# zrjer/Sparse-Matrix-Factorization-Library

Measured on AMD Instinct MI355X. Metric: numeric-factorization GFLOP/s (supernodal Cholesky), higher is better.
Workload: dtype f64; 1 GPU; 3D 7-point Laplacian 128^3 SPD Cholesky fp64, geometric ND, devSlotSize 8694792192; n=2097152, nnz_input=8339456, nsuper=35419, factor_doubles=3787034536, parallelism=single GPU, grid_rule=BASELINE config

## Files before the change

sparse-matrix-factorization-library_amd/csrc/sf_chol_plan.hip:

```cpp
#include <sparseframe_hip.h>

#include <algorithm>
#include <time.h>
#include <cmath>
#include <cstdio>
#include <cstdlib>
#include <cstring>
#include <string>
#include <vector>

#include "sf_plan_internal.h"
#include "sf_symbolic.h"

extern "C" {

int sf_device_count(void) {
    int n = 0;
    if (hipGetDeviceCount(&n) != hipSuccess) return 0;
    return n;
}

size_t sf_device_memory(int device) {
    hipDeviceProp_t prop;
    if (hipGetDeviceProperties(&prop, device) != hipSuccess) return 0;
// ... 199 lines not shown
                if (p->lu) sf::launch_getrf(p->d_potrf + L.first, L.count, p->d_Lsx, p->xC, p->d_info, pc, st);
                else sf::launch_potrf(p->d_potrf + L.first, L.count, p->d_Lsx, p->d_info, st);
                break;
            case 1: sf::launch_trsm(p->d_trsm + L.first, L.count, p->d_Lsx, pc.pivinv, st); break;
            case 7: {
                const int g = (int)L.first;
                const int upto = p->ooc_wait.empty() ? g - 2 : p->ooc_wait[(size_t)g];
                for (int w = std::max(0, g - 2); w <= upto && w < g; ++w) {
                    std::unique_lock<std::mutex> lk(p->dl_mu);
                    p->dl_cv.wait(lk, [&] { return p->dl_abort || p->dl_group_left[(size_t)w].load() <= 0; });
                    if (p->dl_abort) return SF_ERR_HIP;
                }
                if (g >= 2 && p->ooc_buf > 0) {
                    const size_t off = (size_t)(g & 1) * (size_t)p->ooc_buf, nb = (size_t)p->ooc_buf * sizeof(double);
                    HIP_TRY(hipMemsetAsync(p->d_Lsx + off, 0, nb, st));
                    if (p->lu) HIP_TRY(hipMemsetAsync(p->d_Lsx + p->xC + off, 0, nb, st));
                }
                if (p->ooc_top_mode >= 1)
                    for (const auto& z : p->ooc_zero[(size_t)g]) {
                        HIP_TRY(hipMemsetAsync(p->d_Lsx + z.first, 0, (size_t)z.second * sizeof(double), st));
                        if (p->lu) HIP_TRY(hipMemsetAsync(p->d_Lsx + p->xC + z.first, 0, (size_t)z.second * sizeof(double), st));
                    }
                assemble(p->d_loadmask + (size_t)g * (size_t)p->nsuper, st);
                break;
            }
            case 6: {
                int64_t lo, hi;
                launch_window(L, L.count, &lo, &hi);
                sf::launch_update_small(p->d_probs, p->d_stasks + L.first + lo, (int)(hi - lo), p->d_Lsx, p->d_relmap, st);
                break;
            }
            case 5:
                sf::launch_step(p->d_steps + L.first, L.count, p->lu ? 1 : 0, p->d_Lsx, p->d_flags, p->epoch, p->d_info, p->d_tinv,
                                p->d_info + 1 + L.ticket, pc, st);
                break;
            case 2:
            case 3:
            case 4: {
                int64_t w0, w1;
                launch_window(L, L.units, &w0, &w1);
                const uint32_t u0 = (uint32_t)w0, u1 = (uint32_t)w1;
                sf::launch_gemm(p->d_probs, p->d_gtasks + L.first, p->d_ktprefix + L.prefix_first, L.count, u0, u1,
                                L.kind == 3 ? 1 : 0, p->d_Lsx, p->d_relmap, p->gemm_dynamic ? p->d_info + 1 + L.ticket : nullptr, st,
                                (L.whole_tiles && !L.split) ? 1 : 0, 0);
                break;
            }
        }
        if (p->profiling) { kinds.push_back(L.kind); mark(); }
        if (p->dl_active) HIP_TRY(dl_publish(p, li + 1));
    }
    if (last && !p->capturing) HIP_TRY(hipEventRecord(p->ev1, st));
    HIP_TRY(hipGetLastError());
    if (p->profiling) {
        HIP_TRY(hipStreamSynchronize(st));
        if (first) {
            p->last_load_ms = p->last_panel_ms = p->last_update_ms = 0;
            for (double& v : p->last_kind_ms) v = 0;
        }
        float ms = 0;
        if (first && !evs.empty() && elapsed_ms(&ms, p->ev0, evs[0])) p->last_load_ms = ms;
        FILE* dump = nullptr;
        if (const char* path = getenv("SF_PROFILE_DUMP")) dump = fopen(path, first ? "w" : "a");
        if (dump && first) fprintf(dump, "launch,kind,tasks,units,flops,ms\n");
        for (size_t k = 0; k + 1 < evs.size(); ++k) {
            if (!elapsed_ms(&ms, evs[k], evs[k + 1])) continue;
            if (kinds[k] == 3) p->last_update_ms += ms; else if (kinds[k] != 6) p->last_panel_ms += ms;
            p->last_kind_ms[kinds[k]] += ms;
// ... 750 lines not shown

int sf_chol_plan_set_profiling(sf_chol_plan* p, int on) {
    if (!p) return SF_ERR_ARG;
    p->profiling = on != 0;
    return SF_OK;
}

double sf_chol_plan_stat(const sf_chol_plan* p, const char* name) {
    if (!p || !name) return -1;
    const std::string k(name);
    if (k == "levels") return p->nlevels;
    if (k == "last_solve_ms") return p->last_solve_ms;
    if (k == "last_solve_many_ms") return p->last_solve_many_ms;
    if (k == "bytes_solve_many") return (double)p->bytes_solve_many;
    if (k == "solve_many_width") return (double)sf::SVM_W;
    if (k == "bytes_selinv") return (double)p->bytes_selinv;
    if (k == "last_selinv_ms") return p->last_selinv_ms;
    if (k == "flops_selinv") return p->flops_selinv;
    if (k == "selinv_valid") return (p->d_sel && p->sel_gen == p->factor_gen) ? 1.0 : 0.0;
    if (k == "last_refine_iters") return (double)p->last_refine_iters;
    if (k == "last_refine_berr0") return p->last_refine_berr0;
    if (k == "last_refine_berr") return p->last_refine_berr;
    if (k == "last_refine_ms") return p->last_refine_ms;
    if (k == "last_residual_ms") return p->last_residual_ms;
    if (k == "bytes_refine") return (double)p->bytes_refine;
    if (k == "refine_row_entries") return (double)p->rf_entries;
    if (k == "perturbed_pivots") return (double)p->last_perturbed;
    if (k == "pivot_tol") return p->piv_tol;
    if (k == "last_to_host_ms") return p->last_to_host_ms;
    if (k == "download_pieces") return (double)p->dl_pieces.size();
    if (k == "top_doubles") return (double)p->top_size;
    if (k == "stored_doubles") return (double)p->xC;
    if (k == "launches") return (double)p->launches.size();
    if (k == "gemm_tasks") return (double)p->n_gemm_tasks;
    if (k == "update_pairs") return (double)p->n_pairs;
    if (k == "flops_exec") return p->flops_exec;
    if (k == "flops_update") return p->flops_update;
    if (k == "flops_panel_gemm") return p->flops_panel_gemm;
    if (k == "scatter_elems") return p->scatter_elems;
    if (k == "bytes_device") return (double)p->bytes_device;
    if (k == "last_ms") return p->last_ms;
    if (k == "last_load_ms") return p->last_load_ms;
    if (k == "last_panel_ms") return p->last_panel_ms;
    if (k == "last_update_ms") return p->last_update_ms;
    if (k == "last_potrf_ms") return p->last_kind_ms[0];
    if (k == "last_trsm_ms") return p->last_kind_ms[1];
    if (k == "last_inner_gemm_ms") return p->last_kind_ms[2];
    if (k == "last_outer_gemm_ms") return p->last_kind_ms[4];
    if (k == "last_step_ms") return p->last_kind_ms[5];
    if (k == "last_small_update_ms") return p->last_kind_ms[6];
    if (k == "flops_update_small") return p->flops_update_small;
    if (k == "flops_outer_gemm") return p->flops_outer_gemm;
    if (k == "flops_tiles") return p->flops_tiles;
    if (k == "flops_tiles_update") return p->flops_tiles_update;
    return -1;
}

}
```

sparse-matrix-factorization-library_amd/csrc/sf_kernels.h:

```cpp
#pragma once
#include <hip/hip_runtime.h>
#include <cstdint>

#include <cstdlib>
static inline const char* sf_exp_env(const char* name) {
#ifdef SF_EXPERIMENTS
    return getenv(name);
#else
    (void)name;
    return nullptr;
#endif
}

namespace sf {

constexpr int NB = 64;
constexpr int OUTER_NB = 512;
constexpr int TRSM_ROWS = 256;
constexpr int ST_ROWS = 64;
constexpr int GEMM_BM = 128;
constexpr int GEMM_BN = 128;
constexpr int GEMM_BK = 16;
constexpr int GEMM_WAVES = 8;
constexpr int GEMM_THREADS = 64 * GEMM_WAVES;
// ... 33 lines not shown
struct PotrfTask {
    int64_t panel;
    int32_t ld, diag, b;
    int32_t first_col;
};

struct PivotCtl {
    double tol, eps;
    int32_t* pivpos;
    int32_t* pivinv;
    int* nperturb;
};

struct TrsmTask {
    int64_t panel;
    int64_t dpanel;
    int32_t ld, diag, b;
    int32_t row0, nrows;
    int32_t unit;
    int32_t first_col;
    int32_t pad;
};

struct StepTask {
    int64_t panel;
    int64_t xpanel;
    int32_t ld, J, diag, b;
    int32_t row0, nrows;
    int32_t flag;
    int32_t mode;
    int32_t slot;
    int32_t next_b;
    int32_t first_col;
    int32_t pad;
};

void launch_build_loadmap(const int64_t* Lp, const int32_t* Li, int32_t n, const int32_t* Super, const int32_t* SuperMap,
                          const int64_t* Lsip, const int32_t* Lsi, const int64_t* Lsxp, int64_t base, int skip_diag, int64_t* map, hipStream_t st);
void launch_loadmap_drop(const int64_t* drop, int64_t count, int64_t* map, hipStream_t st);
void launch_load_mapped(const double* Lx, const int64_t* map, int64_t nnz, double* Lsx, hipStream_t st);
void launch_load_panels(const int64_t* Lp, const int32_t* Li, const double* Lx, int32_t n,
                        const int32_t* Super, const int32_t* SuperMap, const int64_t* Lsip, const int32_t* Lsi,
                        const int64_t* Lsxp, double* Lsx, int skip_diag, const int8_t* load_mask, hipStream_t st);
void launch_potrf(const PotrfTask* tasks, int ntasks, double* Lsx, int* info, hipStream_t st);
void launch_getrf(const PotrfTask* tasks, int ntasks, double* Lsx, int64_t u_shift, int* info, PivotCtl pc, hipStream_t st);
struct FillTile { int64_t xp; int32_t nsrow, r0, c0, cb, ce; };
void launch_factor_hash(const int32_t* Super, const int64_t* Lsip, const int64_t* Xp, const int64_t* RefXp, int32_t nsuper,
                        const double* PL, const double* PU, int lu, int64_t total, unsigned long long* H, hipStream_t st);
void launch_lu_fill_u11(const FillTile* tiles, int64_t ntiles, double* PL, const double* PU, hipStream_t st);
void launch_pack_lu(const int32_t* Super, const int64_t* Lsip, const int64_t* Xp, const int64_t* RefXp, int32_t nsuper,
                    const double* PL, const double* PU, double* out, int64_t e_begin, int64_t e_end, hipStream_t st);
void launch_trsm(const TrsmTask* tasks, int ntasks, double* Lsx, const int32_t* pivinv, hipStream_t st);
void launch_step(const StepTask* tasks, int ntasks, int lu, double* Lsx, int* flags, int epoch, int* info, double* tinv, int* ticket,
                 PivotCtl pc, hipStream_t st);
void launch_build_relmaps(const GemmProb* probs, int nprobs, const int32_t* Lsi, int32_t* RelMap, hipStream_t st);

void launch_gemm(const GemmProb* probs, const GemmTask* tasks, const uint32_t* kt_prefix, int ntasks, uint32_t u_lo, uint32_t u_hi,
                 int mode, double* Lsx, const int32_t* RelMap, int* ticket, hipStream_t st, int whole_tiles = 0, int grid_cap = 0);

void launch_update_small(const GemmProb* probs, const GemmTask* tasks, int ntasks, double* Lsx, const int32_t* RelMap, hipStream_t st);

struct SolveTask {
    int64_t panel;
    int64_t rows;
    int32_t ld, diag, b;
    int32_t row0, nrows;
    int32_t first_col;
    int32_t flag;
    int32_t expect;
    int64_t tdiag;
};
constexpr int SVM_W = 16;
void launch_solve_small_fwd(const SolveTask* t, int nt, int width, const double* Lsx, const int32_t* Lsi, double* x, int unit,
                            const int32_t* pivpos, hipStream_t st);
void launch_solve_small_bwd(const SolveTask* t, int nt, int width, const double* Lsx, const int32_t* Lsi, double* x, hipStream_t st);
void launch_solve_fwd(const SolveTask* t, int nt, int width, int big, const double* Lsx, const int32_t* Lsi, double* x, int unit,
                      const int32_t* pivpos, int* sync, int* ticket, int* info, hipStream_t st);
void launch_solve_bwd(const SolveTask* t, int nt, int width, int big, const double* Lsx, const int32_t* Lsi, double* x, int* sync, int* ticket,
                      int* info, hipStream_t st, const double* Tbase = nullptr);
void launch_solve_transpose_diag(const SolveTask* tasks, const int64_t* list, int64_t ntasks, const double* Lsx, double* T, hipStream_t st);

void launch_solve_many_pack(const double* Bc, int64_t n, int cw, double* X, hipStream_t st);
void launch_solve_many_unpack(const double* X, int64_t n, int cw, double* Bc, hipStream_t st);

struct SelUnit {
    int64_t lx, rows;
    int32_t nsrow, ncol, cb, w;
// ... 28 lines not shown
```

sparse-matrix-factorization-library_amd/csrc/sf_plan_build.hip:

```cpp
#include <sparseframe_hip.h>

#include <algorithm>
#include <time.h>
#include <cmath>
#include <cstdio>
#include <cstdlib>
#include <cstring>
#include <vector>

#include "sf_plan_internal.h"
#include "sf_symbolic.h"

static thread_local double* t_offer_ptr = nullptr;
static thread_local size_t t_offer_bytes = 0;
extern "C" void sf_plan_offer_factor_buffer(double* ptr, size_t bytes) { t_offer_ptr = ptr; t_offer_bytes = bytes; }

struct PlanInput {
    sf_long n = 0, nsuper = 0;
    const sf_long *Super = nullptr, *SuperMap = nullptr, *Lsip = nullptr, *Lsi = nullptr, *Lsxp = nullptr;
    const sf_long *Lp = nullptr, *Li = nullptr, *Up = nullptr, *Ui = nullptr;
    bool lu = false;
    int device = 0;
    bool dry = false;
    const int32_t* phase_in = nullptr;
    int load_top = 1, rank = 0, nranks = 1;
    const uint32_t* top_mask = nullptr;
    const double* root_cum = nullptr;
    const int32_t* ooc_group = nullptr;
    int ooc_ngroups = 0, ooc_top_mode = 0;

    sf_long nscol(sf_long s) const { return Super[s + 1] - Super[s]; }
    sf_long nsrow(sf_long s) const { return Lsip[s + 1] - Lsip[s]; }
    bool ooc() const { return ooc_group != nullptr && ooc_ngroups > 1; }
    int sides() const { return lu ? 2 : 1; }
};

static bool exp_on(const char* name) {
    const char* env = sf_exp_env(name);
    return !(env && atoi(env) == 0);
}

struct PlanKnobs {
    bool trace = false;
    int su_maxk = sf::SU_MAXK;
    int64_t fuse_max = 32 * sf::GEMM_GRID;
    bool lookahead = true;
    bool use_graph = false;
    bool top_owner = false;
    bool solve_diagT = true, solve_bwd_ahead = true, solve_bwd_fused = true, solve_fwd_ahead = true, solve_fwd_far_first = true;
    int solve_far_wgs = 512, solve_far_groups = 8;
    int dl_workers = DL_WORKERS_DEFAULT, dl_workers_fresh = DL_WORKERS_FRESH;
    bool dl_host_wait = true;
    int64_t dl_slot = DL_SLOT_DEFAULT;
    bool dl_2d = true;
    bool dl_lu_pack = false;
    bool stream_priority = true;
    bool gemm_dynamic = true;
    double piv_tol = 0.0, piv_perturb = 0.0;
};

static PlanKnobs read_knobs() {
    PlanKnobs k;
    k.trace = getenv("SF_TRACE") != nullptr;
    if (const char* env = sf_exp_env("SF_SU_MAXK")) k.su_maxk = atoi(env);
    if (const char* env = getenv("SF_FUSE_MAX")) k.fuse_max = strtoll(env, nullptr, 10);
    if (const char* env = getenv("SF_LOOKAHEAD")) k.lookahead = atoi(env) != 0;
    if (const char* env = getenv("SF_GRAPH")) k.use_graph = atoi(env) != 0;
    if (const char* env = getenv("SF_TOP_OWNER")) k.top_owner = atoi(env) != 0;
    k.solve_diagT = exp_on("SF_SOLVE_DIAGT");
    k.solve_bwd_ahead = exp_on("SF_SOLVE_BWD_AHEAD");
    k.solve_bwd_fused = exp_on("SF_SOLVE_BWD_FUSED");
    k.solve_fwd_ahead = exp_on("SF_SOLVE_FWD_AHEAD");
    k.solve_fwd_far_first = exp_on("SF_SOLVE_FWD_FAR_FIRST");
    if (const char* env = sf_exp_env("SF_SOLVE_FAR_WGS")) k.solve_far_wgs = std::max(1, atoi(env));
    if (const char* env = sf_exp_env("SF_SOLVE_FAR_GROUPS")) k.solve_far_groups = std::max(1, std::min(64, atoi(env)));
    if (const char* env = getenv("SF_DL_WORKERS")) k.dl_workers = k.dl_workers_fresh = std::max(1, std::min(DL_WORKERS_MAX, atoi(env)));
    k.dl_host_wait = exp_on("SF_DL_HOST_WAIT");
    if (const char* env = getenv("SF_DL_SLOT_MB")) k.dl_slot = (int64_t)std::max(1, atoi(env)) << 17;
    k.dl_2d = exp_on("SF_DL_2D");
    if (const char* env = sf_exp_env("SF_DL_LU_PACK")) k.dl_lu_pack = atoi(env) != 0;
    k.stream_priority = exp_on("SF_STREAM_PRIORITY");
    k.gemm_dynamic = exp_on("SF_GEMM_DYNAMIC");
    if (const char* env = getenv("SF_LU_PIVOT_TOL")) {
        k.piv_tol = std::min(1.0, std::max(0.0, atof(env)));
        if (k.piv_tol > 0.0) k.piv_perturb = 1.4901161193847656e-08;
    }
    if (const char* env = getenv("SF_LU_PERTURB")) k.piv_perturb = std::max(0.0, atof(env));
    return k;
}

struct Layout {
    std::vector<int64_t> XP;
    std::vector<uint32_t> gmask;
    int64_t ushift = 0;
    uint32_t all_ranks = 1;
    int rank = 0;
    int group_idx(uint32_t m) const { return __builtin_popcount(m & ((1u << rank) - 1u)); }
};
// ... 400 lines not shown

static void reduce_point(const PlanInput& in, const Layout& lay, const LevelSet& LS, sf_chol_plan& p, int jo, bool ahead) {
    const int J = jo * sf::OUTER_NB;
    if (!p.segments.empty()) p.segments.back().l1 = p.launches.size();
    Segment sg;
    sg.mask = LS.mask;
    sg.l0 = p.launches.size();
    for (sf_long s : LS.sn) {
        const int64_t nscol = in.nscol(s), nsrow = in.nsrow(s);
        if (J >= nscol) continue;
        const int64_t w = std::min<int64_t>(sf::OUTER_NB, nscol - J);
        for (int side = 0; side < in.sides(); ++side) {
            const int64_t base = lay.XP[s] + (side ? lay.ushift : 0);
            sg.off.push_back(base + (int64_t)J * nsrow);
            sg.cnt.push_back(w * nsrow);
            sg.src.push_back(base + (int64_t)J * nsrow + J);
            sg.rows.push_back(nsrow - J);
            sg.cols.push_back(w);
            sg.ld.push_back(nsrow);
            sg.packed += (nsrow - J) * w;
        }
    }
    sg.early = ahead && jo > 0;
    if (p.top_owner && ahead && LS.share_cnt == in.nranks) sg.owner_gi = jo % LS.share_cnt;
    p.segments.push_back(std::move(sg));
}

struct SweepState {
    bool split_set = false;
    int ooc_open = -1;
    std::vector<int32_t> pre_updated;
};

static int fused_step(const PlanInput& in, const Layout& lay, const LevelSet& LS, SweepState& sw, PlanTables& T, sf_chol_plan& p,
                      int jo, int ti, int diag) {
    const bool lu = in.lu;
    const int J = jo * sf::OUTER_NB, ninner = sf::OUTER_NB / sf::NB;
    const int64_t ushift = lay.ushift;
    const std::vector<int64_t>& XP = lay.XP;
    std::vector<StepTask>& steps = T.steps;
    const int64_t d0 = (int64_t)steps.size();
    std::vector<int32_t> flag_of, slot_of;
    for (sf_long s : LS.sn) {
        const int nscol = (int)in.nscol(s), nsrow = (int)in.nsrow(s);
        if (diag >= nscol) { flag_of.push_back(-1); slot_of.push_back(-1); continue; }
        const int b = std::min(sf::NB, nscol - diag);
        flag_of.push_back(T.n_flags);
        if (lu && ti >= 2 && sw.pre_updated[(size_t)s] != jo * 16 + ti) {
            fprintf(stderr, "[sparseframe-hip] plan_create: LU step %d of outer block %d of supernode %lld has no pre-update task\n", ti, jo, (long long)s);
            return SF_ERR_ARG;
        }
        steps.push_back(StepTask{XP[s], XP[s] + (lu ? ushift : 0), nsrow, lu ? (ti >= 2 ? diag - sf::NB : J) : diag, diag, b, diag, b, T.n_flags++, 0, (int32_t)(steps.size() - d0), 0, (int32_t)in.Super[s], 0});
        slot_of.push_back((int32_t)(steps.size() - 1 - d0));
        if (ti > 0) p.flops_panel_gemm += (lu ? 2.0 : 1.0) * ((double)b * (b + 1) * (diag - J) + 2.0 * (nsrow - diag - b) * (double)b * (diag - J));
    }
    if (lu && ti >= 1 && ti + 1 < ninner) {
        const int dnext = diag + sf::NB;
        for (sf_long s : LS.sn) {
            const int nscol = (int)in.nscol(s), nsrow = (int)in.nsrow(s);
            if (dnext >= nscol) continue;
            const int bn = std::min(sf::NB, nscol - dnext);
            steps.push_back(StepTask{XP[s], XP[s] + ushift, nsrow, J, dnext, bn, dnext, bn, -1, 2, 0, 0, (int32_t)in.Super[s], 0});
            sw.pre_updated[(size_t)s] = jo * 16 + ti + 1;
        }
    }
    size_t si = 0;
    for (sf_long s : LS.sn) {
        const int nscol = (int)in.nscol(s), nsrow = (int)in.nsrow(s);
        const int32_t fl = flag_of[si], sl = slot_of[si];
        ++si;
        if (fl < 0) continue;
        const int b = std::min(sf::NB, nscol - diag);
        for (int r = diag + b; r < nsrow; r += sf::ST_ROWS) {
            const int nr = std::min(sf::ST_ROWS, nsrow - r);
            if (!lu) {
                const int nb = (r < std::min(nscol, J + sf::OUTER_NB)) ? std::min(sf::NB, nscol - r) : 0;
                steps.push_back(StepTask{XP[s], XP[s], nsrow, J, diag, b, r, nr, fl, 0, sl, nb, (int32_t)in.Super[s], 0});
            } else {
                steps.push_back(StepTask{XP[s], XP[s] + ushift, nsrow, J, diag, b, r, nr, fl, 0, sl, 0, (int32_t)in.Super[s], 0});
                steps.push_back(StepTask{XP[s] + ushift, XP[s], nsrow, J, diag, b, r, nr, fl, 1, sl, 0, (int32_t)in.Super[s], 0});
            }
        }
    }
    if ((int64_t)steps.size() > d0) {
        p.launches.push_back(Launch{5, d0, (int)(steps.size() - d0)});
        p.launches.back().ticket = p.n_tickets++;
    }
    T.max_diag_tasks = std::max<int64_t>(T.max_diag_tasks, (int64_t)slot_of.size());
    return SF_OK;
}

static void three_launch_step(const PlanInput& in, const Layout& lay, const LevelSet& LS, PlanTables& T, sf_chol_plan& p, int J, int diag) {
    const std::vector<int64_t>& XP = lay.XP;
    const int64_t ushift = lay.ushift;
    const int64_t p0 = (int64_t)T.potrf.size(), t0 = (int64_t)T.trsm.size(), g0 = (int64_t)T.gtasks.size();
    for (sf_long s : LS.sn) {
        const int nscol = (int)in.nscol(s), nsrow = (int)in.nsrow(s);
        if (diag >= nscol) continue;
        const int b = std::min(sf::NB, nscol - diag);
        if (diag > J) {
            GemmProb g{};
            g.lda = nsrow; g.ldc = nsrow;
            g.M = nsrow - diag; g.N = b; g.K = diag - J;
            const int64_t src = XP[s] + diag + (int64_t)J * nsrow;
            const int64_t dst = XP[s] + diag + (int64_t)diag * nsrow;
            const int32_t first = push_sides(in, lay, T, g, src, dst);
            for (int32_t id = first; id < (int32_t)T.probs.size(); ++id) {
                p.flops_panel_gemm += (double)g.N * (g.N + 1) * g.K + 2.0 * (g.M - g.N) * (double)g.N * g.K;
                add_tiles(T, p, id);
            }
        }
        T.potrf.push_back(PotrfTask{XP[s], nsrow, diag, b, (int32_t)in.Super[s]});
        const int below = diag + b;
        for (int r = below; r < nsrow; r += sf::TRSM_ROWS) {
            const int nr = std::min(sf::TRSM_ROWS, nsrow - r);
            if (!in.lu) {
                T.trsm.push_back(TrsmTask{XP[s], XP[s], nsrow, diag, b, r, nr, 0, (int32_t)in.Super[s], 0});
            } else {
                T.trsm.push_back(TrsmTask{XP[s], XP[s] + ushift, nsrow, diag, b, r, nr, 0, (int32_t)in.Super[s], 0});
// ... 78 lines not shown
        p.launches.back().flops = level_small_flops;
    }
}

static int schedule_set(const PlanInput& in, const PlanKnobs& kn, const Layout& lay, const LevelSet& LS, SweepState& sw, PlanTables& T,
                        sf_chol_plan& p) {
    if (LS.ph == 1 && !sw.split_set) { p.launch_split = p.launches.size(); sw.split_set = true; }
    while (in.ooc() && LS.group > sw.ooc_open) p.launches.push_back(Launch{7, (int64_t)++sw.ooc_open, 0});
    const bool shared = set_is_shared(in, LS);
    sf_long maxcol = 0;
    for (sf_long s : LS.sn) maxcol = std::max(maxcol, in.nscol(s));
    const int nouter = (int)((maxcol + sf::OUTER_NB - 1) / sf::OUTER_NB);
    const bool ahead = shared && p.lookahead && LS.share_cnt > 1;
    constexpr int KT_BLOCK = sf::OUTER_NB / sf::GEMM_BK;
    for (int jo = 0; jo < nouter; ++jo) {
        const int J = jo * sf::OUTER_NB;
        if (jo > 0 && !ahead) outer_gemm(in, lay, LS, T, p, J, 0, -1, shared);
        if (shared) {
            reduce_point(in, lay, LS, p, jo, ahead);
            if (ahead && jo > 0) outer_gemm(in, lay, LS, T, p, J, (jo - 1) * KT_BLOCK, jo * KT_BLOCK, false);
        }
        const int ninner = sf::OUTER_NB / sf::NB;
        bool block_fused = false;
        for (int ti = 0; ti < ninner; ++ti) {
            const int diag = J + ti * sf::NB;
            if (diag >= maxcol) break;
            int64_t step_wgs = 0;
            for (sf_long s : LS.sn) {
                const int64_t nscol = in.nscol(s), nsrow = in.nsrow(s);
                if (diag < nscol) step_wgs += 1 + in.sides() * ((nsrow - std::min<int64_t>(nscol, diag + sf::NB) + sf::ST_ROWS - 1) / sf::ST_ROWS);
            }
            if (ti == 0) block_fused = step_wgs <= kn.fuse_max;
            if (!block_fused) three_launch_step(in, lay, LS, T, p, J, diag);
            else if (int rc = fused_step(in, lay, LS, sw, T, p, jo, ti, diag)) return rc;
        }
        const bool owner_block = shared && !p.segments.empty() && p.segments.back().owner_gi >= 0;
        if (owner_block) p.segments.back().lc = p.launches.size();
        for (sf_long s : LS.sn)
            if (J < in.nscol(s)) T.blk_ready[T.blk_first[s] + jo] = p.launches.size() + (owner_block ? 1 : 0);
        if (ahead && jo + 2 < nouter) outer_gemm(in, lay, LS, T, p, J + 2 * sf::OUTER_NB, 0, (jo + 1) * KT_BLOCK, true);
    }
    schur_updates(in, kn, lay, LS, T, p);
    return SF_OK;
}

static int schedule_factorization(const PlanInput& in, const PlanKnobs& kn, const Layout& lay, const std::vector<LevelSet>& sets,
                                  PlanTables& T, sf_chol_plan& p) {
    T.blk_first.assign(in.nsuper + 1, 0);
    for (sf_long s = 0; s < in.nsuper; ++s) T.blk_first[s + 1] = T.blk_first[s] + (in.nscol(s) + sf::OUTER_NB - 1) / sf::OUTER_NB;
    T.blk_ready.assign(T.blk_first[in.nsuper], 0);
    p.lookahead = kn.lookahead;
    p.use_graph = kn.use_graph;
    p.top_owner = kn.top_owner && !in.lu;
    SweepState sw;
    sw.pre_updated.assign(in.lu ? (size_t)std::max<sf_long>(in.nsuper, 1) : 0, -1);
    p.launch_split = 0;
    for (const LevelSet& LS : sets)
        if (int rc = schedule_set(in, kn, lay, LS, sw, T, p)) return rc;
    if (!sw.split_set) p.launch_split = p.launches.size();
    if (!p.segments.empty()) p.segments.back().l1 = p.launches.size();
    p.n_gemm_tasks = (int64_t)T.gtasks.size() + (int64_t)T.stasks.size();
    return SF_OK;
}

static void schedule_solve(const PlanInput& in, const PlanKnobs& kn, const Layout& lay, PlanTables& T, sf_chol_plan& p) {
    int32_t n_solve_sync = 0;
    const bool solve_mapped = p.partial && in.top_mask != nullptr && in.load_top == 2;
// ... 745 lines not shown
```

sparse-matrix-factorization-library_amd/csrc/sf_plan_internal.h:

```cpp
#pragma once
#include <sparseframe_hip.h>

#include <algorithm>
#include <atomic>
#include <condition_variable>
#include <cstdio>
#include <cstdlib>
#include <memory>
#include <mutex>
#include <thread>
#include <utility>
#include <vector>

#include "sf_kernels.h"

using sf::GemmProb;
using sf::GemmTask;
using sf::PotrfTask;
using sf::TrsmTask;
using sf::StepTask;

struct Launch {
    int kind;
    int64_t first;
    int count;
    int64_t prefix_first = 0;
    uint32_t units = 0;
    double flops = 0;
    bool split = false;
    int share_idx = 0, share_cnt = 1;
    bool whole_tiles = false;
    double share_lo = 0.0, share_hi = 1.0;
    int ticket = 0;
};

struct Segment {
    uint32_t mask = 0;
    size_t l0 = 0, l1 = 0;
    std::vector<int64_t> off, cnt;
    std::vector<int64_t> src, rows, cols, ld;
    int64_t packed = 0;
    bool early = false;
    int owner_gi = -1;
    size_t lc = 0;
};

#define HIP_TRY(expr)                                                                       \
    do {                                                                                    \
        hipError_t e_ = (expr);                                                             \
        if (e_ != hipSuccess) {                                                             \
            fprintf(stderr, "[sparseframe-hip] %s failed: %s (%s:%d)\n", #expr, hipGetErrorString(e_), __FILE__, __LINE__); \
            return SF_ERR_HIP;                                                              \
        }                                                                                   \
    } while (0)

template <class T>
static inline int upload(T** dptr, const std::vector<T>& h, size_t* bytes_total) {
    *dptr = nullptr;
    const size_t bytes = std::max<size_t>(h.size(), 1) * sizeof(T);
    HIP_TRY(hipMalloc((void**)dptr, bytes));
    if (!h.empty()) HIP_TRY(hipMemcpy(*dptr, h.data(), h.size() * sizeof(T), hipMemcpyHostToDevice));
    *bytes_total += bytes;
    return SF_OK;
}

constexpr int64_t DL_SLOT_DEFAULT = (int64_t)4 << 20;
// ... 142 lines not shown
    std::vector<SelStep> sel_steps;
    std::vector<sf::SelPair> sel_pairs_h;
    int64_t sel_linv_elems = 0, sel_y_elems = 0, sel_z_elems = 0, sel_s_elems = 0;
    double* d_sel = nullptr;
    double* d_sel_diag = nullptr;
    void* d_sel_units = nullptr;
    void* d_sel_pairs = nullptr;
    double* d_sel_scratch = nullptr;
    size_t bytes_selinv = 0;
    double last_selinv_ms = 0, flops_selinv = 0;
    int64_t *d_rf_ptr = nullptr, *d_rf_pos = nullptr, *d_rf_cptr = nullptr, *d_rf_cpos = nullptr;
    int32_t *d_rf_col = nullptr, *d_rf_ccol = nullptr;
    double* d_rf_vec = nullptr;
    int64_t rf_entries = 0, rf_anorm_gen = -1;
    size_t bytes_refine = 0;
    int last_refine_iters = 0;
    double last_refine_berr0 = 0, last_refine_berr = 0, last_refine_ms = 0, last_residual_ms = 0;
    int device = 0;
    int64_t n = 0, nsuper = 0, nnz = 0, isize = 0, xsize = 0;
    hipStream_t stream = nullptr;
    hipEvent_t ev0 = nullptr, ev1 = nullptr, ev_s0 = nullptr, ev_s1 = nullptr;

    int64_t* d_Lp = nullptr;
    int32_t* d_Li = nullptr;
    double* d_Lx = nullptr;
    int32_t* d_Super = nullptr;
    int32_t* d_SuperMap = nullptr;
    int64_t* d_Lsip = nullptr;
    int32_t* d_Lsi = nullptr;
    int64_t* d_Lsxp = nullptr;
    double* d_Lsx = nullptr;
    int* d_info = nullptr;
    int n_tickets = 0;
    bool gemm_dynamic = true;

    PotrfTask* d_potrf = nullptr;
    TrsmTask* d_trsm = nullptr;
    StepTask* d_steps = nullptr;
    int* d_flags = nullptr;
    double* d_tinv = nullptr;
    int epoch = 0;
    std::vector<uint64_t> h_hash;
    int hash_epoch = -1;
    GemmProb* d_probs = nullptr;
    GemmTask* d_gtasks = nullptr;
    GemmTask* d_stasks = nullptr;
    uint32_t* d_ktprefix = nullptr;
    int32_t* d_relmap = nullptr;

    std::vector<Launch> launches;
    int nlevels = 0;
    int64_t n_gemm_tasks = 0, n_pairs = 0;
    double flops_tiles = 0, flops_tiles_update = 0;
    double flops_update_small = 0;
    double flops_exec = 0, flops_update = 0, scatter_elems = 0, flops_panel_gemm = 0, flops_outer_gemm = 0;
    size_t bytes_device = 0;
    bool values_set = false;

    bool profiling = false;
    double last_ms = 0, last_load_ms = 0, last_panel_ms = 0, last_update_ms = 0;
    double last_kind_ms[8] = {0, 0, 0, 0, 0, 0, 0, 0};
    int last_status = SF_OK;

    std::vector<int64_t> h_Lsip, h_Lsxp;
    std::vector<int32_t> h_Super;
    std::vector<int> level_of;
// ... 16 lines not shown
```

sparse-matrix-factorization-library_amd/csrc/sf_step.hip:

```cpp
#include "sf_kernels.h"
#include "sf_panel.h"
#include "sf_wave.h"

namespace sf {

#ifndef SF_LU_STEP_WGS
#define SF_LU_STEP_WGS 3
#endif
#ifndef SF_POTRF_PW
#define SF_POTRF_PW 16
#endif
constexpr int ST_ULD = ST_ROWS + 1;
constexpr int ST_KC = 32;
constexpr int ST_XLD = ST_ROWS + 16;
constexpr int ST_SPIN_LIMIT = 1 << 22;

constexpr int ST_SMEM = 2 * ST_KC * ST_XLD;
static_assert(NB == ST_ROWS && NB == 64, "one wavefront per 64 x 64 tile");
static_assert(NB * ST_ULD <= ST_SMEM && NB * NB + 4 * 256 <= ST_SMEM, "phases must fit the LDS array");

struct StepCtx {
    StepTask t;
    int tid, lane, wave;
    int fr, fk;
    int64_t ld;
    int b, nrows;
    double* Ag;
    const double* Dg;
    bool is_diag;
};

#ifdef SF_EXP_STEP_STAMPS
__device__ unsigned long long* g_step_stamps = nullptr;
void exp_set_step_stamps(unsigned long long* p) { (void)hipMemcpyToSymbol(HIP_SYMBOL(g_step_stamps), &p, sizeof(p)); }
#define ST_STAMP(slot) do { if (c.is_diag && c.tid == 0 && g_step_stamps) g_step_stamps[slot] = wall_clock64(); } while (0)
#else
#define ST_STAMP(slot) do { } while (0)
#endif

__device__ __forceinline__ double ld_agent(const double* p) {
    return __hip_atomic_load(p, __ATOMIC_RELAXED, __HIP_MEMORY_SCOPE_AGENT);
}
__device__ __forceinline__ int ld_agent(const int* p) {
    return __hip_atomic_load(p, __ATOMIC_RELAXED, __HIP_MEMORY_SCOPE_AGENT);
}

#define ST_FOR_EACH_ACC(q, r) _Pragma("unroll") for (int q = 0; q < 4; ++q) _Pragma("unroll") for (int r = 0; r < 4; ++r)
#define ST_ACC_ROW (16 * c.wave + c.fr)
#define ST_ACC_COL(q, r) (16 * (q) + c.fk + 4 * (r))

__device__ __forceinline__ void step_update(const StepCtx& c, const double* Lsx, double (*Xs)[ST_KC][ST_XLD], int nhp, double4_t (&acc)[4]) {
    const StepTask& t = c.t;
    const int tid = c.tid, wave = c.wave, fr = c.fr, fk = c.fk, b = c.b, nrows = c.nrows;
    const int64_t ld = c.ld;
    const int nch = 2 * nhp;
    const int prow = 2 * (tid & 31), pk0 = tid >> 5;
    const double* __restrict__ xp = Lsx + t.xpanel + t.diag + (int64_t)t.J * ld + ((prow < b) ? prow : 0);
    const double* __restrict__ yp = Lsx + t.panel + t.row0 + (int64_t)(t.J + fk) * ld + min(16 * wave + fr, nrows - 1);
    const int nhalf = 2 * nch;
    double2_t rx[2][4];
    double fy[4][4];
    auto load_x = [&](int sel, int h) __attribute__((always_inline)) {
        const int hc = min(h, nch - 1);
#pragma unroll
        for (int q = 0; q < 4; ++q) rx[sel][q] = *reinterpret_cast<const double2_t*>(xp + (int64_t)(hc * ST_KC + pk0 + 8 * q) * ld);
    };
    auto store_x = [&](int buf, int sel) __attribute__((always_inline)) {
#pragma unroll
        for (int q = 0; q < 4; ++q) *reinterpret_cast<double2_t*>(&Xs[buf][pk0 + 8 * q][prow]) = rx[sel][q];
    };
    auto load_y = [&](int slot, int hh) __attribute__((always_inline)) {
        const int hc = min(hh, nhalf - 1);
#pragma unroll
        for (int kk = 0; kk < 4; ++kk) fy[slot][kk] = yp[(int64_t)(hc * (ST_KC / 2) + 4 * kk) * ld];
    };
    auto compute = [&](int par, int h) __attribute__((always_inline)) {
        load_y((2 * par + 3) & 3, 2 * h + 3);
#pragma unroll
        for (int kk = 0; kk < 8; ++kk) {
            double a[4];
#pragma unroll
            for (int q = 0; q < 4; ++q) a[q] = Xs[par][4 * kk + fk][16 * q + fr];
            if (kk == 0) store_x(par ^ 1, par ^ 1);
            if (kk == 1) load_x(par ^ 1, h + 3);
            if (kk == 4) load_y(2 * par, 2 * h + 4);
#pragma unroll
            for (int q = 0; q < 4; ++q) acc[q] = __builtin_amdgcn_mfma_f64_16x16x4f64(a[q], fy[2 * par + (kk >> 2)][kk & 3], acc[q], 0, 0, 0);
        }
    };
    load_x(0, 0);
    load_x(1, 1);
    load_y(0, 0);
    load_y(1, 1);
    load_y(2, 2);
    store_x(0, 0);
    load_x(0, 2);
    __syncthreads();
    for (int hp = 0; hp < nhp; ++hp) {
        compute(0, 2 * hp);
        __syncthreads();
        compute(1, 2 * hp + 1);
        __syncthreads();
    }
}

__device__ __forceinline__ void step_pre_store(const StepCtx& c, double* Lsx, const double4_t (&acc)[4]) {
    const StepTask& t = c.t;
    const int b = c.b;
    const int64_t ld = c.ld;
    double* Ag = c.Ag;
    double* __restrict__ Dw = Lsx + t.xpanel + t.diag + (int64_t)t.diag * ld;
    const int ci = ST_ACC_ROW;
    ST_FOR_EACH_ACC(q, r) {
        const int cj = ST_ACC_COL(q, r);
        const int cic = min(ci, b - 1), cjc = min(cj, b - 1);
        const double dl = Ag[cic + (int64_t)cjc * ld], du = Dw[cjc + (int64_t)cic * ld];
        if (ci < b && cj < b) {
            if (cj < ci) Ag[ci + (int64_t)cj * ld] = dl - acc[q][r];
            else Dw[cj + (int64_t)ci * ld] = du - acc[q][r];
        }
// ... 285 lines not shown
    if (c.tid == 0) {
        int spins = 0;
        while (__hip_atomic_load(flags + flag, __ATOMIC_RELAXED, __HIP_MEMORY_SCOPE_AGENT) != epoch) {
            __builtin_amdgcn_s_sleep(16);
            if (++spins > ST_SPIN_LIMIT) { atomicOr(info, 2); break; }
        }
#ifdef SF_EXP_ACQUIRE_FENCE
        __builtin_amdgcn_fence(__ATOMIC_ACQUIRE, "agent");
#endif
        asm volatile("s_waitcnt vmcnt(0)" ::: "memory");
    }
    __syncthreads();
}

__device__ __forceinline__ void step_permute_cols(const StepCtx& c, const int32_t* pivinv, double* U, double4_t (&rt)[4]) {
    const int b = c.b;
    const int g0 = c.t.first_col + c.t.diag;
    int src[16];
    bool ident = true;
    ST_FOR_EACH_ACC(q, r) {
        const int cj = ST_ACC_COL(q, r);
        src[4 * q + r] = (cj < b) ? ld_agent(pivinv + g0 + cj) - g0 : cj;
        ident = ident && src[4 * q + r] == cj;
    }
    if (!__all(ident)) {
        const int ci = ST_ACC_ROW;
        ST_FOR_EACH_ACC(q, r) U[ST_ACC_COL(q, r) * ST_ULD + ci] = rt[q][r];
        ST_FOR_EACH_ACC(q, r) rt[q][r] = U[src[4 * q + r] * ST_ULD + ci];
    }
    __syncthreads();
}

template <bool LU>
__device__ __forceinline__ void step_row_solve(const StepCtx& c, const double* tinv, double (*Dt)[NB], double* Tl, bool park, double4_t (&rt)[4]) {
    const StepTask& t = c.t;
    const int tid = c.tid, wave = c.wave, fr = c.fr, fk = c.fk, b = c.b, nrows = c.nrows;
    const int64_t ld = c.ld;
    double* Ag = c.Ag;
    const double* Dg = c.Dg;
    const double* __restrict__ tsrc = tinv + (int64_t)t.slot * (LU ? 2048 : 1024) + ((LU && (t.mode & 1)) ? 1024 : 0);
    {
        double dv[NB * NB / 256], tv[4];
#pragma unroll
        for (int i = 0; i < NB * NB / 256; ++i) {
            const int e = tid + 256 * i, k = e / NB, j = e % NB;
            dv[i] = ld_agent(Dg + min(j, b - 1) + (int64_t)min(k, b - 1) * ld);
        }
#pragma unroll
        for (int i = 0; i < 4; ++i) tv[i] = ld_agent(tsrc + tid + 256 * i);
#pragma unroll
        for (int i = 0; i < NB * NB / 256; ++i) {
            const int e = tid + 256 * i, k = e / NB, j = e % NB;
            Dt[k][j] = (j < b && k < j) ? dv[i] : 0.0;
        }
#pragma unroll
        for (int i = 0; i < 4; ++i) Tl[tid + 256 * i] = tv[i];
    }
    __syncthreads();
    const int ci = 16 * wave + fr;
#pragma unroll
    for (int q = 0; q < 4; ++q) {
        if (16 * q >= b) break;
        double4_t x = (double4_t){0.0, 0.0, 0.0, 0.0};
#pragma unroll
        for (int sg = 0; sg < 4; ++sg)
            x = __builtin_amdgcn_mfma_f64_16x16x4f64(Tl[q * 256 + (4 * sg + fk) * 16 + fr], rt[q][sg], x, 0, 0, 0);
#pragma unroll
        for (int qq = q + 1; qq < 4; ++qq)
#pragma unroll
            for (int sg = 0; sg < 4; ++sg)
                rt[qq] = __builtin_amdgcn_mfma_f64_16x16x4f64(-Dt[16 * q + 4 * sg + fk][16 * qq + fr], x[sg], rt[qq], 0, 0, 0);
#pragma unroll
        for (int r = 0; r < 4; ++r) {
            const int cj = 16 * q + fk + 4 * r;
            if (ci < nrows && cj < b) Ag[ci + (int64_t)cj * ld] = x[r];
        }
        if (park) {
            __syncthreads();
#pragma unroll
            for (int r = 0; r < 4; ++r) Dt[16 * q + fk + 4 * r][ci] = x[r];
        }
    }
}

__device__ __forceinline__ void step_push_next(const StepCtx& c, double* Lsx, double (*Dt)[NB]) {
    const StepTask& t = c.t;
    const int wave = c.wave, fr = c.fr, fk = c.fk;
    const int64_t ld = c.ld;
    const int ci = 16 * wave + fr;
    __syncthreads();
    double* __restrict__ Dn = Lsx + t.panel + t.row0 + (int64_t)t.row0 * ld;
    const int nb = t.next_b;
    for (int ct = 0; ct <= wave; ++ct) {
        double4_t d = (double4_t){0.0, 0.0, 0.0, 0.0};
#pragma unroll 4
        for (int sg = 0; sg < 16; ++sg)
            d = __builtin_amdgcn_mfma_f64_16x16x4f64(Dt[4 * sg + fk][16 * ct + fr], Dt[4 * sg + fk][ci], d, 0, 0, 0);
        double old[4];
#pragma unroll
        for (int r = 0; r < 4; ++r) {
            const int cj = 16 * ct + fk + 4 * r;
            old[r] = Dn[min(ci, nb - 1) + (int64_t)min(cj, nb - 1) * ld];
        }
#pragma unroll
        for (int r = 0; r < 4; ++r) {
            const int cj = 16 * ct + fk + 4 * r;
            if (ci < nb && cj <= ci) Dn[ci + (int64_t)cj * ld] = old[r] - d[r];
        }
    }
}

template <bool LU>
__global__ void __launch_bounds__(256, LU ? SF_LU_STEP_WGS : 3)
k_step(const StepTask* __restrict__ tasks, double* __restrict__ Lsx, int* __restrict__ flags, int epoch, int* __restrict__ info,
       double* __restrict__ tinv, int* __restrict__ ticket, PivotCtl pc) {
    __shared__ __attribute__((aligned(16))) double smem[ST_SMEM];
    double (*Xs)[ST_KC][ST_XLD] = reinterpret_cast<double (*)[ST_KC][ST_XLD]>(smem);
    double* U = smem;
    double (*Dt)[NB] = reinterpret_cast<double (*)[NB]>(smem);
    double* Tl = smem + NB * NB;

    __shared__ int s_ticket;
    const int tid = threadIdx.x, lane = tid & 63, wave = tid >> 6;
#ifdef SF_EXP_STEP_STAMPS
    const unsigned long long st_entry = wall_clock64();
#endif
    if (tid == 0) s_ticket = __hip_atomic_fetch_add(ticket, 1, __ATOMIC_RELAXED, __HIP_MEMORY_SCOPE_AGENT);
    __syncthreads();
    const StepTask t = tasks[__builtin_amdgcn_readfirstlane(s_ticket)];
    const bool is_pre = LU && (t.mode & 2);
    const bool is_diag = t.row0 == t.diag && !is_pre;
    const StepCtx c = {t, tid, lane, wave, lane & 15, lane >> 4, t.ld, t.b, t.nrows,
                       Lsx + t.panel + t.row0 + (int64_t)t.diag * t.ld, Lsx + t.xpanel + t.diag + (int64_t)t.diag * t.ld, is_diag};
#ifdef SF_EXP_STEP_STAMPS
    if (is_diag && tid == 0 && g_step_stamps) g_step_stamps[0] = st_entry;
#endif
    ST_STAMP(1);

    double4_t acc[4];
#pragma unroll
    for (int a = 0; a < 4; ++a) acc[a] = (double4_t){0.0, 0.0, 0.0, 0.0};
    const int nhp = ((is_pre ? t.diag - NB : t.diag) - t.J) / NB;
    if (nhp > 0) step_update(c, Lsx, Xs, nhp, acc);

    if (is_pre) {
        step_pre_store(c, Lsx, acc);
        return;
    }
    double4_t rt[4];
    if (!is_diag) step_row_tile(c, acc, rt);
    if (is_diag) {
        if constexpr (LU) {
            __shared__ int s_piv[NB], s_pos[NB];
            step_diag_lu(c, Lsx, U, s_piv, s_pos, nhp > 0, acc, info, tinv, pc);
        } else {
            step_diag_chol(c, U, acc, info, tinv);
        }
        step_publish(c, flags, t.flag, epoch);
        ST_STAMP(9);
        return;
    }

    step_wait(c, flags, t.flag, epoch, info);
    if (LU && (t.mode & 1) && pc.pivinv) step_permute_cols(c, pc.pivinv, U, rt);
    const bool push = !LU && t.next_b > 0;
    step_row_solve<LU>(c, tinv, Dt, Tl, push, rt);
    if (push) step_push_next(c, Lsx, Dt);
}

void launch_step(const StepTask* tasks, int ntasks, int lu, double* Lsx, int* flags, int epoch, int* info, double* tinv, int* ticket,
                 PivotCtl pc, hipStream_t st) {
    if (ntasks <= 0) return;
    if (lu) hipLaunchKernelGGL(k_step<true>, dim3(ntasks), dim3(256), 0, st, tasks, Lsx, flags, epoch, info, tinv, ticket, pc);
    else hipLaunchKernelGGL(k_step<false>, dim3(ntasks), dim3(256), 0, st, tasks, Lsx, flags, epoch, info, tinv, ticket, pc);
}

}
```

Baseline: 55780 GFLOP/s.

## Pair adjacent row tiles in fused step kernel for large launches

When a fused step launch has more tasks than a threshold, off-diagonal row tiles with no next-block push are merged in pairs. One workgroup then computes two 64-row tiles, reusing the loaded X panel and the triangular inverse for both and halving the number of workgroups. A separate wide kernel variant with launch bounds of 2 waves per SIMD holds the doubled accumulators. The cost is more register pressure, lower occupancy and fewer workgroups to spread across CUs.

```diff
diff --git a/sparse-matrix-factorization-library_amd/csrc/sf_chol_plan.hip b/sparse-matrix-factorization-library_amd/csrc/sf_chol_plan.hip
--- a/sparse-matrix-factorization-library_amd/csrc/sf_chol_plan.hip
+++ b/sparse-matrix-factorization-library_amd/csrc/sf_chol_plan.hip
@@ -255,7 +255,7 @@
             }
             case 5:
                 sf::launch_step(p->d_steps + L.first, L.count, p->lu ? 1 : 0, p->d_Lsx, p->d_flags, p->epoch, p->d_info, p->d_tinv,
-                                p->d_info + 1 + L.ticket, pc, st);
+                                p->d_info + 1 + L.ticket, pc, st, L.wide ? 1 : 0);
                 break;
             case 2:
             case 3:
@@ -1072,6 +1072,12 @@
     if (k == "top_doubles") return (double)p->top_size;
     if (k == "stored_doubles") return (double)p->xC;
     if (k == "launches") return (double)p->launches.size();
+    if (k == "step_launches" || k == "step_wide_launches") {
+        double cnt = 0;
+        for (const Launch& L : p->launches) cnt += (L.kind == 5 && (L.wide || k == "step_launches")) ? 1 : 0;
+        return cnt;
+    }
+    if (k == "step_pairs") return (double)p->n_step_pairs;
     if (k == "gemm_tasks") return (double)p->n_gemm_tasks;
     if (k == "update_pairs") return (double)p->n_pairs;
     if (k == "flops_exec") return p->flops_exec;
diff --git a/sparse-matrix-factorization-library_amd/csrc/sf_kernels.h b/sparse-matrix-factorization-library_amd/csrc/sf_kernels.h
--- a/sparse-matrix-factorization-library_amd/csrc/sf_kernels.h
+++ b/sparse-matrix-factorization-library_amd/csrc/sf_kernels.h
@@ -89,7 +89,7 @@
     int32_t slot;
     int32_t next_b;
     int32_t first_col;
-    int32_t pad;
+    int32_t pair;
 };
 
 void launch_build_loadmap(const int64_t* Lp, const int32_t* Li, int32_t n, const int32_t* Super, const int32_t* SuperMap,
@@ -109,7 +109,7 @@
                     const double* PL, const double* PU, double* out, int64_t e_begin, int64_t e_end, hipStream_t st);
 void launch_trsm(const TrsmTask* tasks, int ntasks, double* Lsx, const int32_t* pivinv, hipStream_t st);
 void launch_step(const StepTask* tasks, int ntasks, int lu, double* Lsx, int* flags, int epoch, int* info, double* tinv, int* ticket,
-                 PivotCtl pc, hipStream_t st);
+                 PivotCtl pc, hipStream_t st, int wide = 0);
 void launch_build_relmaps(const GemmProb* probs, int nprobs, const int32_t* Lsi, int32_t* RelMap, hipStream_t st);
 
 void launch_gemm(const GemmProb* probs, const GemmTask* tasks, const uint32_t* kt_prefix, int ntasks, uint32_t u_lo, uint32_t u_hi,
diff --git a/sparse-matrix-factorization-library_amd/csrc/sf_plan_build.hip b/sparse-matrix-factorization-library_amd/csrc/sf_plan_build.hip
--- a/sparse-matrix-factorization-library_amd/csrc/sf_plan_build.hip
+++ b/sparse-matrix-factorization-library_amd/csrc/sf_plan_build.hip
@@ -40,10 +40,13 @@
     return !(env && atoi(env) == 0);
 }
 
+constexpr int64_t STEP_PAIR_MIN_DEFAULT = 1536;
+
 struct PlanKnobs {
     bool trace = false;
     int su_maxk = sf::SU_MAXK;
     int64_t fuse_max = 32 * sf::GEMM_GRID;
+    int64_t step_pair_min = STEP_PAIR_MIN_DEFAULT;
     bool lookahead = true;
     bool use_graph = false;
     bool top_owner = false;
@@ -64,6 +67,7 @@
     k.trace = getenv("SF_TRACE") != nullptr;
     if (const char* env = sf_exp_env("SF_SU_MAXK")) k.su_maxk = atoi(env);
     if (const char* env = getenv("SF_FUSE_MAX")) k.fuse_max = strtoll(env, nullptr, 10);
+    if (const char* env = getenv("SF_STEP_PAIR_MIN")) k.step_pair_min = strtoll(env, nullptr, 10);
     if (const char* env = getenv("SF_LOOKAHEAD")) k.lookahead = atoi(env) != 0;
     if (const char* env = getenv("SF_GRAPH")) k.use_graph = atoi(env) != 0;
     if (const char* env = getenv("SF_TOP_OWNER")) k.top_owner = atoi(env) != 0;
@@ -530,8 +534,8 @@
     std::vector<int32_t> pre_updated;
 };
 
-static int fused_step(const PlanInput& in, const Layout& lay, const LevelSet& LS, SweepState& sw, PlanTables& T, sf_chol_plan& p,
-                      int jo, int ti, int diag) {
+static int fused_step(const PlanInput& in, const PlanKnobs& kn, const Layout& lay, const LevelSet& LS, SweepState& sw, PlanTables& T,
+                      sf_chol_plan& p, int jo, int ti, int diag) {
     const bool lu = in.lu;
     const int J = jo * sf::OUTER_NB, ninner = sf::OUTER_NB / sf::NB;
     const int64_t ushift = lay.ushift;
@@ -562,6 +566,12 @@
             sw.pre_updated[(size_t)s] = jo * 16 + ti + 1;
         }
     }
+    int64_t ntasks64 = (int64_t)steps.size() - d0;
+    for (sf_long s : LS.sn) {
+        const int64_t nscol = in.nscol(s), nsrow = in.nsrow(s);
+        if (diag < nscol) ntasks64 += in.sides() * ((nsrow - std::min<int64_t>(nscol, diag + sf::NB) + sf::ST_ROWS - 1) / sf::ST_ROWS);
+    }
+    const bool wide = ntasks64 > kn.step_pair_min;
     size_t si = 0;
     for (sf_long s : LS.sn) {
         const int nscol = (int)in.nscol(s), nsrow = (int)in.nsrow(s);
@@ -569,20 +579,24 @@
         ++si;
         if (fl < 0) continue;
         const int b = std::min(sf::NB, nscol - diag);
-        for (int r = diag + b; r < nsrow; r += sf::ST_ROWS) {
+        for (int r = diag + b; r < nsrow;) {
             const int nr = std::min(sf::ST_ROWS, nsrow - r);
+            const int nb = (!lu && r < std::min(nscol, J + sf::OUTER_NB)) ? std::min(sf::NB, nscol - r) : 0;
+            const int32_t pair = (wide && nb == 0 && r + 2 * sf::ST_ROWS <= nsrow) ? sf::ST_ROWS : 0;
             if (!lu) {
-                const int nb = (r < std::min(nscol, J + sf::OUTER_NB)) ? std::min(sf::NB, nscol - r) : 0;
-                steps.push_back(StepTask{XP[s], XP[s], nsrow, J, diag, b, r, nr, fl, 0, sl, nb, (int32_t)in.Super[s], 0});
+                steps.push_back(StepTask{XP[s], XP[s], nsrow, J, diag, b, r, nr, fl, 0, sl, nb, (int32_t)in.Super[s], pair});
             } else {
-                steps.push_back(StepTask{XP[s], XP[s] + ushift, nsrow, J, diag, b, r, nr, fl, 0, sl, 0, (int32_t)in.Super[s], 0});
-                steps.push_back(StepTask{XP[s] + ushift, XP[s], nsrow, J, diag, b, r, nr, fl, 1, sl, 0, (int32_t)in.Super[s], 0});
-            }
+                steps.push_back(StepTask{XP[s], XP[s] + ushift, nsrow, J, diag, b, r, nr, fl, 0, sl, 0, (int32_t)in.Super[s], pair});
+                steps.push_back(StepTask{XP[s] + ushift, XP[s], nsrow, J, diag, b, r, nr, fl, 1, sl, 0, (int32_t)in.Super[s], pair});
+            }
+            r += sf::ST_ROWS + pair;
+            if (pair) p.n_step_pairs += in.sides();
         }
     }
     if ((int64_t)steps.size() > d0) {
         p.launches.push_back(Launch{5, d0, (int)(steps.size() - d0)});
         p.launches.back().ticket = p.n_tickets++;
+        p.launches.back().wide = wide;
     }
     T.max_diag_tasks = std::max<int64_t>(T.max_diag_tasks, (int64_t)slot_of.size());
     return SF_OK;
@@ -727,7 +741,7 @@
             }
             if (ti == 0) block_fused = step_wgs <= kn.fuse_max;
             if (!block_fused) three_launch_step(in, lay, LS, T, p, J, diag);
-            else if (int rc = fused_step(in, lay, LS, sw, T, p, jo, ti, diag)) return rc;
+            else if (int rc = fused_step(in, kn, lay, LS, sw, T, p, jo, ti, diag)) return rc;
         }
         const bool owner_block = shared && !p.segments.empty() && p.segments.back().owner_gi >= 0;
         if (owner_block) p.segments.back().lc = p.launches.size();
diff --git a/sparse-matrix-factorization-library_amd/csrc/sf_plan_internal.h b/sparse-matrix-factorization-library_amd/csrc/sf_plan_internal.h
--- a/sparse-matrix-factorization-library_amd/csrc/sf_plan_internal.h
+++ b/sparse-matrix-factorization-library_amd/csrc/sf_plan_internal.h
@@ -32,6 +32,7 @@
     bool whole_tiles = false;
     double share_lo = 0.0, share_hi = 1.0;
     int ticket = 0;
+    bool wide = false;
 };
 
 struct Segment {
@@ -240,6 +241,7 @@
     double* d_Lsx = nullptr;
     int* d_info = nullptr;
     int n_tickets = 0;
+    int64_t n_step_pairs = 0;
     bool gemm_dynamic = true;
 
     PotrfTask* d_potrf = nullptr;
diff --git a/sparse-matrix-factorization-library_amd/csrc/sf_step.hip b/sparse-matrix-factorization-library_amd/csrc/sf_step.hip
--- a/sparse-matrix-factorization-library_amd/csrc/sf_step.hip
+++ b/sparse-matrix-factorization-library_amd/csrc/sf_step.hip
@@ -49,7 +49,9 @@
 #define ST_ACC_ROW (16 * c.wave + c.fr)
 #define ST_ACC_COL(q, r) (16 * (q) + c.fk + 4 * (r))
 
-__device__ __forceinline__ void step_update(const StepCtx& c, const double* Lsx, double (*Xs)[ST_KC][ST_XLD], int nhp, double4_t (&acc)[4]) {
+template <int NT>
+__device__ __forceinline__ void step_update(const StepCtx& c, const double* Lsx, double (*Xs)[ST_KC][ST_XLD], int nhp, double4_t (&acc)[NT][4],
+                                            int nrows2 = 0) {
     const StepTask& t = c.t;
     const int tid = c.tid, wave = c.wave, fr = c.fr, fk = c.fk, b = c.b, nrows = c.nrows;
     const int64_t ld = c.ld;
@@ -57,9 +59,10 @@
     const int prow = 2 * (tid & 31), pk0 = tid >> 5;
     const double* __restrict__ xp = Lsx + t.xpanel + t.diag + (int64_t)t.J * ld + ((prow < b) ? prow : 0);
     const double* __restrict__ yp = Lsx + t.panel + t.row0 + (int64_t)(t.J + fk) * ld + min(16 * wave + fr, nrows - 1);
+    const int yoff2 = (NT > 1) ? ST_ROWS + min(16 * wave + fr, nrows2 - 1) - min(16 * wave + fr, nrows - 1) : 0;
     const int nhalf = 2 * nch;
     double2_t rx[2][4];
-    double fy[4][4];
+    double fy[NT][4][4];
     auto load_x = [&](int sel, int h) __attribute__((always_inline)) {
         const int hc = min(h, nch - 1);
 #pragma unroll
@@ -72,7 +75,11 @@
     auto load_y = [&](int slot, int hh) __attribute__((always_inline)) {
         const int hc = min(hh, nhalf - 1);
 #pragma unroll
-        for (int kk = 0; kk < 4; ++kk) fy[slot][kk] = yp[(int64_t)(hc * (ST_KC / 2) + 4 * kk) * ld];
+        for (int kk = 0; kk < 4; ++kk) {
+            const double* __restrict__ y = yp + (int64_t)(hc * (ST_KC / 2) + 4 * kk) * ld;
+            fy[0][slot][kk] = y[0];
+            if constexpr (NT > 1) fy[1][slot][kk] = y[yoff2];
+        }
     };
     auto compute = [&](int par, int h) __attribute__((always_inline)) {
         load_y((2 * par + 3) & 3, 2 * h + 3);
@@ -85,7 +92,9 @@
             if (kk == 1) load_x(par ^ 1, h + 3);
             if (kk == 4) load_y(2 * par, 2 * h + 4);
 #pragma unroll
-            for (int q = 0; q < 4; ++q) acc[q] = __builtin_amdgcn_mfma_f64_16x16x4f64(a[q], fy[2 * par + (kk >> 2)][kk & 3], acc[q], 0, 0, 0);
+            for (int n = 0; n < NT; ++n)
+#pragma unroll
+                for (int q = 0; q < 4; ++q) acc[n][q] = __builtin_amdgcn_mfma_f64_16x16x4f64(a[q], fy[n][2 * par + (kk >> 2)][kk & 3], acc[n][q], 0, 0, 0);
         }
     };
     load_x(0, 0);
@@ -437,11 +446,10 @@
 }
 
 template <bool LU>
-__device__ __forceinline__ void step_row_solve(const StepCtx& c, const double* tinv, double (*Dt)[NB], double* Tl, bool park, double4_t (&rt)[4]) {
+__device__ __forceinline__ void step_row_load(const StepCtx& c, const double* tinv, double (*Dt)[NB], double* Tl) {
     const StepTask& t = c.t;
-    const int tid = c.tid, wave = c.wave, fr = c.fr, fk = c.fk, b = c.b, nrows = c.nrows;
-    const int64_t ld = c.ld;
-    double* Ag = c.Ag;
+    const int tid = c.tid, b = c.b;
+    const int64_t ld = c.ld;
     const double* Dg = c.Dg;
     const double* __restrict__ tsrc = tinv + (int64_t)t.slot * (LU ? 2048 : 1024) + ((LU && (t.mode & 1)) ? 1024 : 0);
     {
@@ -462,6 +470,12 @@
         for (int i = 0; i < 4; ++i) Tl[tid + 256 * i] = tv[i];
     }
     __syncthreads();
+}
+
+__device__ __forceinline__ void step_row_solve(const StepCtx& c, double (*Dt)[NB], double* Tl, bool park, double4_t (&rt)[4]) {
+    const int wave = c.wave, fr = c.fr, fk = c.fk, b = c.b, nrows = c.nrows;
+    const int64_t ld = c.ld;
+    double* Ag = c.Ag;
     const int ci = 16 * wave + fr;
 #pragma unroll
     for (int q = 0; q < 4; ++q) {
@@ -516,9 +530,34 @@
 }
 
 template <bool LU>
-__global__ void __launch_bounds__(256, LU ? SF_LU_STEP_WGS : 3)
-k_step(const StepTask* __restrict__ tasks, double* __restrict__ Lsx, int* __restrict__ flags, int epoch, int* __restrict__ info,
-       double* __restrict__ tinv, int* __restrict__ ticket, PivotCtl pc) {
+__device__ __forceinline__ void step_row_pair(const StepCtx& c, const double* Lsx, double (*Xs)[ST_KC][ST_XLD], double* U, double (*Dt)[NB],
+                                              double* Tl, int nhp, int* flags, int epoch, int* info, const double* tinv, const PivotCtl& pc) {
+    StepCtx c2 = c;
+    c2.t.row0 += ST_ROWS;
+    c2.nrows = c.t.pair;
+    c2.Ag += ST_ROWS;
+    double4_t acc[2][4];
+#pragma unroll
+    for (int n = 0; n < 2; ++n)
+#pragma unroll
+        for (int a = 0; a < 4; ++a) acc[n][a] = (double4_t){0.0, 0.0, 0.0, 0.0};
+    if (nhp > 0) step_update<2>(c, Lsx, Xs, nhp, acc, c2.nrows);
+    double4_t rt[2][4];
+    step_row_tile(c, acc[0], rt[0]);
+    step_row_tile(c2, acc[1], rt[1]);
+    step_wait(c, flags, c.t.flag, epoch, info);
+    if (LU && (c.t.mode & 1) && pc.pivinv) {
+        step_permute_cols(c, pc.pivinv, U, rt[0]);
+        step_permute_cols(c2, pc.pivinv, U, rt[1]);
+    }
+    step_row_load<LU>(c, tinv, Dt, Tl);
+    step_row_solve(c, Dt, Tl, false, rt[0]);
+    step_row_solve(c2, Dt, Tl, false, rt[1]);
+}
+
+template <bool LU, bool WIDE>
+__device__ __forceinline__ void step_body(const StepTask* __restrict__ tasks, double* __restrict__ Lsx, int* __restrict__ flags, int epoch,
+                                          int* __restrict__ info, double* __restrict__ tinv, int* __restrict__ ticket, const PivotCtl& pc) {
     __shared__ __attribute__((aligned(16))) double smem[ST_SMEM];
     double (*Xs)[ST_KC][ST_XLD] = reinterpret_cast<double (*)[ST_KC][ST_XLD]>(smem);
     double* U = smem;
@@ -542,11 +581,18 @@
 #endif
     ST_STAMP(1);
 
-    double4_t acc[4];
+    double4_t acc1[1][4];
+    double4_t (&acc)[4] = acc1[0];
 #pragma unroll
     for (int a = 0; a < 4; ++a) acc[a] = (double4_t){0.0, 0.0, 0.0, 0.0};
     const int nhp = ((is_pre ? t.diag - NB : t.diag) - t.J) / NB;
-    if (nhp > 0) step_update(c, Lsx, Xs, nhp, acc);
+    if constexpr (WIDE) {
+        if (t.pair > 0) {
+            step_row_pair<LU>(c, Lsx, Xs, U, Dt, Tl, nhp, flags, epoch, info, tinv, pc);
+            return;
+        }
+    }
+    if (nhp > 0) step_update<1>(c, Lsx, Xs, nhp, acc1);
 
     if (is_pre) {
         step_pre_store(c, Lsx, acc);
@@ -569,13 +615,33 @@
     step_wait(c, flags, t.flag, epoch, info);
     if (LU && (t.mode & 1) && pc.pivinv) step_permute_cols(c, pc.pivinv, U, rt);
     const bool push = !LU && t.next_b > 0;
-    step_row_solve<LU>(c, tinv, Dt, Tl, push, rt);
+    step_row_load<LU>(c, tinv, Dt, Tl);
+    step_row_solve(c, Dt, Tl, push, rt);
     if (push) step_push_next(c, Lsx, Dt);
 }
 
+template <bool LU>
+__global__ void __launch_bounds__(256, LU ? SF_LU_STEP_WGS : 3)
+k_step(const StepTask* __restrict__ tasks, double* __restrict__ Lsx, int* __restrict__ flags, int epoch, int* __restrict__ info,
+       double* __restrict__ tinv, int* __restrict__ ticket, PivotCtl pc) {
+    step_body<LU, false>(tasks, Lsx, flags, epoch, info, tinv, ticket, pc);
+}
+
+template <bool LU>
+__global__ void __launch_bounds__(256, 2)
+k_step_wide(const StepTask* __restrict__ tasks, double* __restrict__ Lsx, int* __restrict__ flags, int epoch, int* __restrict__ info,
+            double* __restrict__ tinv, int* __restrict__ ticket, PivotCtl pc) {
+    step_body<LU, true>(tasks, Lsx, flags, epoch, info, tinv, ticket, pc);
+}
+
 void launch_step(const StepTask* tasks, int ntasks, int lu, double* Lsx, int* flags, int epoch, int* info, double* tinv, int* ticket,
-                 PivotCtl pc, hipStream_t st) {
+                 PivotCtl pc, hipStream_t st, int wide) {
     if (ntasks <= 0) return;
+    if (wide) {
+        if (lu) hipLaunchKernelGGL(k_step_wide<true>, dim3(ntasks), dim3(256), 0, st, tasks, Lsx, flags, epoch, info, tinv, ticket, pc);
+        else hipLaunchKernelGGL(k_step_wide<false>, dim3(ntasks), dim3(256), 0, st, tasks, Lsx, flags, epoch, info, tinv, ticket, pc);
+        return;
+    }
     if (lu) hipLaunchKernelGGL(k_step<true>, dim3(ntasks), dim3(256), 0, st, tasks, Lsx, flags, epoch, info, tinv, ticket, pc);
     else hipLaunchKernelGGL(k_step<false>, dim3(ntasks), dim3(256), 0, st, tasks, Lsx, flags, epoch, info, tinv, ticket, pc);
 }
```

New measurement: 55600 GFLOP/s. Within noise of the previous version (-0.3%).
